# gear-genomics/tracy

Hardware: AMD Instinct MI355X
Metric: GCUPS (tracy align: Gotoh affine-gap DP cells per second, whole job) (higher is better)
Workload: dtype int16 (score sweeps) / int32 (tracebacks)

## Files before the change

### tracy_amd/csrc/capi.hip

```cpp
#include <hip/hip_runtime.h>
#include <atomic>
#include <sched.h>
#include <malloc.h>
#include <map>
#include <chrono>

#include <thread>

#include <algorithm>
#include <cctype>
#include <cstdarg>
#include <cstddef>
#include <cstdio>
#include <cstdlib>
#include <cstring>
#include <string>
#include <memory>
#include <vector>

#include "../../include/tracy_hip.h"
#include "capi_internal.h"
#include "launch.h"
#include "stream_plan.h"
#include "sweep_range.h"
// ... 196 lines not shown
  if (!p.on) return;
  const double ms = (double)(now_ns() - t0) * 1e-6;
  std::lock_guard<std::mutex> lk(p.m);
  auto& e = p.acc[label];
  e.first += ms;
  e.second += 1;
}

namespace {
struct KnobField { const char* name; bool CtxKnobs::*flag; };
const KnobField kKnobFlags[] = {
    {"no_stream", &CtxKnobs::no_stream}, {"no_narrow", &CtxKnobs::no_narrow}, {"no_compact", &CtxKnobs::no_compact},
    {"no_screen", &CtxKnobs::no_screen}, {"no_band", &CtxKnobs::no_band}, {"no_band16", &CtxKnobs::no_band16},
    {"no_front", &CtxKnobs::no_front}, {"no_prefix", &CtxKnobs::no_prefix}, {"no_vote", &CtxKnobs::no_vote},
    {"no_origin", &CtxKnobs::no_origin}, {"no_subwindow", &CtxKnobs::no_subwindow}, {"no_prelim_origin", &CtxKnobs::no_prelim_origin},
    {"no_cq", &CtxKnobs::no_cq}, {"no_fused_walk", &CtxKnobs::no_fused_walk}, {"no_cont16", &CtxKnobs::no_cont16}, {"no_decomp_wave", &CtxKnobs::no_decomp_wave}, {"no_af_split", &CtxKnobs::no_af_split}, {"no_front_lists", &CtxKnobs::no_front_lists}, {"no_origin_band", &CtxKnobs::no_origin_band}, {"no_quads", &CtxKnobs::no_quads}, {"no_fork", &CtxKnobs::no_fork}, {"no_early_tail", &CtxKnobs::no_early_tail}, {"sweeps_alone", &CtxKnobs::sweeps_alone}, {"no_sweep_diag", &CtxKnobs::no_sweep_diag}, {"verbose", &CtxKnobs::verbose}};
bool same_name(const char* a, const char* b) {
  for (; *a && *b; ++a, ++b)
    if (std::tolower((unsigned char)*a) != std::tolower((unsigned char)*b)) return false;
  return *a == *b;
}
}
bool knobs_set(CtxKnobs& k, const char* name, const char* value) {
  if (!name || !value) return false;
  if (same_name(name, "band_w")) {
    char* end = nullptr;
    const long v = strtol(value, &end, 10);
    if (end == value) return false;
    k.band_w = v < 0 ? -1 : (int32_t)std::min<long>(4096, v);
    return true;
  }
  if (same_name(name, "quad_tier_min")) {
    const long v = atol(value);
    if (v < 0) return false;
    k.quad_tier_min = (uint32_t)std::min<long>(v, 0x7fffffffl);
    return true;
  }
  if (same_name(name, "front_list_min")) {
    const long v = atol(value);
    if (v < 0) return false;
    k.front_list_min = (uint32_t)std::min<long>(v, 0x7fffffffl);
    return true;
  }
  if (same_name(name, "b16_multi_max")) {
    char* end = nullptr;
    const long v = strtol(value, &end, 10);
    if (end == value || *end || v < 0 || v > 0x7fffffffl) return false;
    k.b16_multi_max = (uint32_t)v;
    return true;
  }
  if (same_name(name, "chain_prio")) {
    if (value[0] < '0' || value[0] > '2' || value[1]) return false;
// ... 29 lines not shown
      return true;
    }
  return false;
}
void knobs_from_env(CtxKnobs& k) {
  for (const KnobField& f : kKnobFlags) {
    std::string env = "TRACYHIP_";
    for (const char* c = f.name; *c; ++c) env.push_back((char)std::toupper((unsigned char)*c));
    if (getenv(env.c_str())) k.*(f.flag) = true;
  }
  if (getenv("TRACYHIP_HOST_TIMERS")) k.verbose = true;
  if (const char* e = getenv("TRACYHIP_BAND_W")) knobs_set(k, "band_w", e);
  if (const char* e = getenv("TRACYHIP_CKPT_B")) knobs_set(k, "ckpt_b", e);
  if (const char* e = getenv("TRACYHIP_QUAD_TIER_MIN")) knobs_set(k, "quad_tier_min", e);
  if (const char* e = getenv("TRACYHIP_FRONT_LIST_MIN")) knobs_set(k, "front_list_min", e);
  if (const char* e = getenv("TRACYHIP_B16_MULTI_MAX")) knobs_set(k, "b16_multi_max", e);
  if (const char* e = getenv("TRACYHIP_CHAIN_PRIO")) knobs_set(k, "chain_prio", e);
  if (const char* e = getenv("TRACYHIP_SEED_VOTE_CAP")) knobs_set(k, "seed_vote_cap", e);
  if (const char* e = getenv("TRACYHIP_SEED_SPILL")) knobs_set(k, "seed_spill", e);
  if (const char* e = getenv("TRACYHIP_SWEEP_DIAG_PERIOD")) knobs_set(k, "sweep_diag_period", e);
}
std::string knobs_describe(const CtxKnobs& k) {
  std::string s;
  for (const KnobField& f : kKnobFlags) { s += f.name; s += k.*(f.flag) ? "=1\n" : "=0\n"; }
  s += "band_w=" + std::to_string(k.band_w) + "\n";
  s += "ckpt_b=" + std::to_string(k.ckpt_b) + "\n";
  s += "quad_tier_min=" + std::to_string(k.quad_tier_min) + "\n";
  s += "front_list_min=" + std::to_string(k.front_list_min) + "\n";
  s += "b16_multi_max=" + std::to_string(k.b16_multi_max) + "\n";
  s += "chain_prio=" + std::to_string(k.chain_prio) + "\n";
  s += "seed_vote_cap=" + std::to_string(k.seed_vote_cap) + "\n";
  s += k.seed_spill ? "seed_spill=1\n" : "seed_spill=0\n";
  s += "sweep_diag_period=" + std::to_string(k.sweep_diag_period) + "\n";
  s += "host_threads=" + std::to_string(host_pool_threads()) + "\n";
  return s;
}

int timing_begin(tracyhip_ctx* ctx, int which, uint64_t cells, uint64_t bytes) {
  if (!ctx->timing) return TRACYHIP_OK;
  tracyhip_ctx::Pending p{which, nullptr, nullptr, cells, bytes};
  HIP_TRY(get_event(ctx, &p.e0));
  HIP_TRY(get_event(ctx, &p.e1));
  HIP_TRY(hipEventRecord(p.e0, ctx->stream));
// ... 702 lines not shown
      b += (uint64_t)kFrontRows + pre[i].n + 4ull * pre[i].n;
    }
    cells[tid] = c; bytes[tid] = b;
  });
  HIP_TRY(ctx->dev[DB_PRE].ensure(sizeof(PairDesc) * np));
  HIP_TRY(hipMemcpyAsync(ctx->dev[DB_PRE].p, hd, sizeof(PairDesc) * np, hipMemcpyHostToDevice, st));
  DpArgs a = scoring_args(ctx, prm);
  a.pairs = static_cast<const PairDesc*>(ctx->dev[DB_PRE].p);
  a.a1 = d_a1; a.a2 = d_a2; a.scores = nullptr;
  a.special_blocks = d_special;
  a.lastrow = d_lastrow;
  uint64_t tc = 0, tb = 0;
  for (uint32_t t = 0; t < kHostThreads; ++t) { tc += cells[t]; tb += bytes[t]; }
  int trc;
  if ((trc = timing_begin(ctx, TRACYHIP_TIMER_SCORE, tc, tb))) return trc;
  HIP_TRY(launch_gotoh_front_prefix_cq(a, (uint32_t)np, st));
  if ((trc = timing_end(ctx))) return trc;
  return TRACYHIP_OK;
}

static int run_front_once(tracyhip_ctx* ctx, const std::vector<FrontDesc>& fd, const int16_t* d_qp, const uint32_t* d_row, const tracyhip_params* prm,
                          FrontResult& out, const uint8_t* d_codes, bool keep_err, int KB, int32_t halfw) {
  hipStream_t st = ctx->stream;
  const size_t nf = fd.size();
  out.fo.assign(nf, FrontOut{});
  out.score.assign(nf, 0);
  out.ce.assign(nf, 0);
  if (nf == 0) return TRACYHIP_OK;
  const size_t per = sizeof(FrontDesc) + sizeof(PairDesc) + sizeof(FrontOut) + sizeof(int32_t) + 2 * sizeof(uint32_t);
  HIP_TRY(ctx->dev[DB_FRONT].ensure(per * nf + 64));
  PairDesc* d_pairs = static_cast<PairDesc*>(ctx->dev[DB_FRONT].p);
// ... 201 lines not shown
    const uint32_t npre = pre_done ? 0u : (uint32_t)np;
    const uint32_t prows = front_shape ? kFrontRows : (uint32_t)kPrefixLanes * (uint32_t)K;
    uint32_t maxm = 0;
    if (ctx->timing) {
      uint64_t cells = 0, bytes = 0;
      for (size_t i = lo; i < hi; ++i) { cells += (uint64_t)hd[i].m * hd[i].n; bytes += 24ull * hd[i].m + hd[i].n + 4; }
      for (size_t i = 0; i < npre; ++i) cells += (uint64_t)std::min<uint32_t>(hd[nf + i].m, prows) * hd[nf + i].n;
      if ((trc = timing_begin(ctx, TRACYHIP_TIMER_SCORE, cells, bytes))) return trc;
    }
    for (size_t i = lo; i < hi; ++i) { maxm = std::max(maxm, hd[i].m); max_mn = std::max<uint64_t>(max_mn, (uint64_t)hd[i].m + hd[i].n); }
    for (size_t i = 0; i < npre; ++i) max_mn = std::max<uint64_t>(max_mn, (uint64_t)hd[nf + i].m + hd[nf + i].n);
    DpArgs af = a;
    af.pairs = static_cast<const PairDesc*>(ctx->dev[DB_DESC].p) + lo;
    DpArgs apl = ap;
    launch_diag_periods(ctx, prm, K, (uint32_t)(hi - lo), npre, front_shape, af, apl);
    if (front_shape) HIP_TRY(launch_gotoh_ckpt_front(K, af, (uint32_t)(hi - lo), apl, npre, st));
    else HIP_TRY(launch_gotoh_ckpt_prefix(K, af, (uint32_t)(hi - lo), apl, npre, st));
    if ((trc = timing_end(ctx))) return trc;
    if (hi > lo) narrow_launches.emplace_back(maxm, narrow_launch_diag(K, af.diag_period));
    if (npre) narrow_launches.emplace_back(prows, narrow_launch_diag(front_shape ? kFrontPrefixK : K, apl.diag_period));
    pre_done = true;
    lo = hi;
  }
  int32_t herr[kErrWords] = {};
  HIP_TRY(hipMemcpyAsync(herr, ctx->dev[DB_ERR].p, sizeof(herr), hipMemcpyDeviceToHost, st));
  HIP_TRY(ctx_sync(ctx));
  timing_collect(ctx);
  return range_verdict(prm, herr, narrow_launches, max_mn, 0);
}
}

// ... 458 lines not shown
```

### tracy_amd/csrc/capi_internal.h

```cpp
#ifndef TRACY_AMD_CAPI_INTERNAL_H
#define TRACY_AMD_CAPI_INTERNAL_H

#include <hip/hip_runtime.h>

#include <atomic>
#include <condition_variable>
#include <deque>
#include <functional>
#include <mutex>
#include <string>
#include <thread>
#include <utility>
#include <vector>

#include "../../include/tracy_hip.h"
#include "assemble_wave.h"
#include "dp_kernels.h"
#include "band16_launch.h"
#include "front.h"

namespace tracyhip {

struct DevBuf {
  void* p = nullptr;
// ... 185 lines not shown
  bool no_sweep_diag = false;
  bool no_origin_band = false;
  bool no_front_lists = false;
  bool no_af_split = false;
  bool no_decomp_wave = false;
  bool no_cont16 = false;
  bool verbose = false;
  int32_t band_w = -1;
  uint32_t ckpt_b = 256;
  uint32_t chain_prio = 1;
  uint32_t sweep_diag_period = 0;
  uint32_t b16_multi_max = TRACY_B16_MULTI_MAX;
  uint32_t front_list_min = 1024;
  uint32_t seed_vote_cap = 2048;
  bool seed_spill = false;
  uint32_t quad_tier_min = 32768;
};
void knobs_from_env(CtxKnobs& k);
bool knobs_set(CtxKnobs& k, const char* name, const char* value);
std::string knobs_describe(const CtxKnobs& k);

constexpr size_t kCodePad = 128;
int choose_k(uint32_t m, int mode, bool needle = false);
uint64_t seqset_extent(const tracyhip_seqset& s);

struct DpProblem {
  int mode = MODE_CHAR;
  bool a1_profile = false, a2_profile = false;
  const void* d_a1 = nullptr;
  const void* d_a2 = nullptr;
// ... 259 lines not shown
```

### tracy_amd/csrc/dp_kernels.hip

```cpp
#include <hip/hip_runtime.h>

#include <cstdlib>

#include "dp_kernels.h"
#include "launch.h"

namespace tracyhip {

static uint32_t lds_pad() {
  static int v = -1;
  if (v < 0) { const char* e = getenv("TRACYHIP_LDS_PAD"); v = e ? atoi(e) : 0; }
  return (uint32_t)v;
}

struct DeviceWave {
  __device__ __forceinline__ uint32_t lane() const { return threadIdx.x; }
  __device__ __forceinline__ int32_t shift_up(int32_t x) const {
    return __builtin_amdgcn_update_dpp(0, x, 0x138, 0xf, 0xf, true);
  }
  __device__ __forceinline__ int32_t shift_up_row(int32_t x) const {
    return __builtin_amdgcn_update_dpp(0, x, 0x111, 0xf, 0xf, true);
  }
  __device__ __forceinline__ int32_t shift_up_or(int32_t x, int32_t first) const {
    return __builtin_amdgcn_update_dpp(first, x, 0x138, 0xf, 0xf, false);
// ... 487 lines not shown
    if (full.special_blocks) {                                                                                          \
      hipLaunchKernelGGL((gotoh_ckpt_prefix_kernel<KK, GL, true>), grid, dim3(64), lds_combo(KK, true), s, full, nfull, pre, npre); \
      hipLaunchKernelGGL((gotoh_ckpt_prefix_kernel<KK, GL, false>), grid, dim3(64), lds_combo(KK, false), s, full, nfull, pre, npre); \
    } else {                                                                                                            \
      hipLaunchKernelGGL((gotoh_ckpt_prefix_kernel<KK, GL, false>), grid, dim3(64), lds_combo(KK, false), s, full, nfull, pre, npre); \
    }                                                                                                                   \
    break;
  switch (K) {
    TRACY_COMBO_CASE(4) TRACY_COMBO_CASE(8) TRACY_COMBO_CASE(12) TRACY_COMBO_CASE(15) TRACY_COMBO_CASE(16)
    default: return hipErrorInvalidValue;
  }
#undef TRACY_COMBO_CASE
  return hipGetLastError();
}

static uint32_t front_prefix_tall_min() {
  static const uint32_t v = [] { const char* e = getenv("TRACYHIP_PREFIX_TALL_MIN"); return e ? (uint32_t)strtoul(e, nullptr, 10) : 40000u; }();
  return v;
}
template <int GL, int KP>
static hipError_t launch_gotoh_ckpt_front_t(int K, const DpArgs& full, uint32_t nfull, const DpArgs& pre, uint32_t npre, hipStream_t s) {
  static_assert(GL * KP == (int)kFrontRows, "the rows above the kept one");
  const dim3 grid(nfull + (npre + 64 / GL - 1) / (64 / GL));
  auto lds = [](int KK, bool compact) {
    const uint32_t pre_b = lds_bytes_prefix(KP, compact), sw = lds_bytes_sweep16(KK, compact);
    return (pre_b > sw ? pre_b : sw) + lds_pad();
  };
#define TRACY_FRONT_CASE(KK)                                                                                            \
  case KK:                                                                                                              \
    if constexpr (KK == 15 || KK == 16) {                                                                               \
      if (combo_uses_diag<KK>(full, nfull, pre, npre)) {                                                                \
        if (full.special_blocks)                                                                                        \
          hipLaunchKernelGGL((gotoh_ckpt_prefix_kernel<KK, GL, true, KP, true>), grid, dim3(64), lds(KK, true), s, full, nfull, pre, npre); \
        hipLaunchKernelGGL((gotoh_ckpt_prefix_kernel<KK, GL, false, KP, true>), grid, dim3(64), lds(KK, false), s, full, nfull, pre, npre); \
// ... 4 lines not shown
       \
       \
      hipLaunchKernelGGL((gotoh_ckpt_prefix_kernel<KK, GL, true, KP>), grid, dim3(64), lds(KK, true), s, full, nfull, pre, npre); \
      hipLaunchKernelGGL((gotoh_ckpt_prefix_kernel<KK, GL, false, KP>), grid, dim3(64), lds(KK, false), s, full, nfull, pre, npre); \
    } else {                                                                                                            \
      hipLaunchKernelGGL((gotoh_ckpt_prefix_kernel<KK, GL, false, KP>), grid, dim3(64), lds(KK, false), s, full, nfull, pre, npre); \
    }                                                                                                                   \
    break;
  switch (K) {
    TRACY_FRONT_CASE(4) TRACY_FRONT_CASE(8) TRACY_FRONT_CASE(12) TRACY_FRONT_CASE(15) TRACY_FRONT_CASE(16)
    default: return hipErrorInvalidValue;
  }
#undef TRACY_FRONT_CASE
  return hipGetLastError();
}
hipError_t launch_gotoh_ckpt_front(int K, const DpArgs& full, uint32_t nfull, const DpArgs& pre, uint32_t npre, hipStream_t s) {
  if (nfull + npre == 0) return hipSuccess;
  if (nfull == 0 && npre >= front_prefix_tall_min()) return launch_gotoh_ckpt_front_t<(int)kFrontRows / 16, 16>(K, full, nfull, pre, npre, s);
  return launch_gotoh_ckpt_front_t<kFrontPrefixLanes, kFrontPrefixK>(K, full, nfull, pre, npre, s);
}

hipError_t launch_gotoh_prefix(int K, const DpArgs& a, uint32_t npairs, hipStream_t s) {
  if (npairs == 0) return hipSuccess;
  constexpr int GL = kPrefixLanes;
  const dim3 grid((npairs + 64 / GL - 1) / (64 / GL));
#define TRACY_PREFIX_CASE(KK) \
  case KK:                                                                                                                      \
    hipLaunchKernelGGL((gotoh_prefix_kernel<KK, GL, false>), grid, dim3(64), lds_bytes_prefix(KK, false), s, a, npairs);                        \
    if (a.special_blocks) hipLaunchKernelGGL((gotoh_prefix_kernel<KK, GL, true>), grid, dim3(64), lds_bytes_prefix(KK, true), s, a, npairs); \
    break;
  switch (K) {
    TRACY_PREFIX_CASE(4) TRACY_PREFIX_CASE(8) TRACY_PREFIX_CASE(12) TRACY_PREFIX_CASE(15) TRACY_PREFIX_CASE(16)
    default: return hipErrorInvalidValue;
  }
#undef TRACY_PREFIX_CASE
  return hipGetLastError();
}
template <int GL, int KP>
static hipError_t launch_gotoh_front_prefix_cq_t(const DpArgs& a, uint32_t npairs, hipStream_t s) {
  const dim3 grid((npairs + 64 / GL - 1) / (64 / GL));
  hipLaunchKernelGGL((gotoh_prefix_kernel<KP, GL, false, true>), grid, dim3(64), lds_bytes_prefix(KP, false), s, a, npairs);
  if (a.special_blocks) hipLaunchKernelGGL((gotoh_prefix_kernel<KP, GL, true, true>), grid, dim3(64), lds_bytes_prefix(KP, true), s, a, npairs);
  return hipGetLastError();
}
hipError_t launch_gotoh_front_prefix_cq(const DpArgs& a, uint32_t npairs, hipStream_t s) {
  if (npairs == 0) return hipSuccess;
  if (npairs >= front_prefix_tall_min()) return launch_gotoh_front_prefix_cq_t<(int)kFrontRows / 16, 16>(a, npairs, s);
  return launch_gotoh_front_prefix_cq_t<kFrontPrefixLanes, kFrontPrefixK>(a, npairs, s);
}
hipError_t launch_gotoh_walk(const WalkArgs& a, hipStream_t s) {
  if (a.npairs == 0) return hipSuccess;
  hipLaunchKernelGGL(gotoh_walk_kernel, dim3(a.npairs), dim3(64), 0, s, a);
  return hipGetLastError();
}
hipError_t launch_needle_walk(const WalkArgs& a, const uint32_t* bits32, hipStream_t s) {
  if (a.npairs == 0) return hipSuccess;
  hipLaunchKernelGGL(needle_walk_kernel, dim3((a.npairs + 63) / 64), dim3(64), 0, s, a, bits32);
  return hipGetLastError();
}
hipError_t launch_alignment_rows(const RowsArgs& a, hipStream_t s) {
  if (a.npairs == 0) return hipSuccess;
  hipLaunchKernelGGL(alignment_rows_kernel, dim3(a.npairs), dim3(64), 0, s, a);
// ... 5 lines not shown
```

### tracy_amd/csrc/launch.h

```cpp
#ifndef TRACY_AMD_LAUNCH_H
#define TRACY_AMD_LAUNCH_H

#include <hip/hip_runtime.h>

#include "dp_kernels.h"

namespace tracyhip {

struct RowsArgs {
  const PairDesc* pairs;
  const void* a1;
  const void* a2;
  int32_t a1_profile, a2_profile;
  int32_t a2_revcomp_flag;
  int32_t a2_onehot;
  const uint8_t* ops;
  const uint64_t* ops_off;
  const uint32_t* ops_len;
  uint8_t* rows0;
  uint8_t* rows1;
  uint32_t npairs;
  const int32_t* row0_gaps_only;
  uint32_t row0_gaps_only_stride;
};

hipError_t launch_gotoh(int mode, int K, bool trace, bool narrow, const DpArgs& a, uint32_t npairs, hipStream_t s, bool rawtab = false);
hipError_t launch_gotoh_front_prefix_cq(const DpArgs& a, uint32_t npairs, hipStream_t s);
hipError_t launch_gotoh_prof(int K, bool trace, bool row4_zero, bool arith16, const DpArgs& a, uint32_t npairs, hipStream_t s);
hipError_t launch_gotoh_ckpt(int mode, int K, bool narrow, const DpArgs& a, uint32_t npairs, hipStream_t s);
hipError_t launch_band_trace(int mode, int K, const DpArgs& a, const WalkArgs& wa, uint32_t npairs, hipStream_t s);
hipError_t launch_gotoh_origin(int K, int table, int codes, const DpArgs& a, uint32_t npairs, hipStream_t s);
hipError_t launch_gotoh_ckpt_prefix(int K, const DpArgs& full, uint32_t nfull, const DpArgs& pre, uint32_t npre, hipStream_t s);
hipError_t launch_gotoh_prefix(int K, const DpArgs& a, uint32_t npairs, hipStream_t s);
hipError_t launch_gotoh_ckpt_front(int K, const DpArgs& full, uint32_t nfull, const DpArgs& pre, uint32_t npre, hipStream_t s);
hipError_t launch_needle(int mode, int K, bool trace, const DpArgs& a, uint32_t npairs, hipStream_t s);
hipError_t launch_gotoh_walk(const WalkArgs& a, hipStream_t s);
hipError_t launch_needle_walk(const WalkArgs& a, const uint32_t* bits32, hipStream_t s);
hipError_t launch_alignment_rows(const RowsArgs& a, hipStream_t s);

}
#endif
```

### tracy_amd/csrc/stream.hip

```cpp
#include <hip/hip_runtime.h>

#include <algorithm>
#include <cstring>
#include <numeric>
#include <string>
#include <type_traits>
#include <vector>

#include "../../include/tracy_hip.h"
#include "capi_internal.h"
#include "decompose_launch.h"
#include "launch.h"
#include "pipe_internal.h"
#include "pipe_kernels.h"
#include "stream_fields.h"
#include "stream_plan.h"

using namespace tracyhip;

#define TRY(expr) do { const int _rc = (expr); if (_rc) return _rc; } while (0)

namespace {

struct Arena {
// ... 236 lines not shown
      q.n = sw.n;
      q.a2_stride = sw.n;
      q.a2_off = G.ref_off + (S.rc ? (uint64_t)(G.rn - ce) : (uint64_t)sw.a);
      q.flags = S.rc ? PAIR_A2_REVCOMP : 0u;
      q.out = t;
      q.ckpt_off = band_pack(sw.dlo, sw.dhi);
      q.lastrow_off = mode == 0 ? 0ull : ((uint64_t)(G.rn - ce) | ((uint64_t)sw.a << 32));
      cand[t] = q;
      kc[t] = (uint8_t)K;
    }
  }
  tr[t] = S;
  if (dd) dead[t] |= dd;
}

constexpr uint32_t kScanBlock = 256, kScanTop = 1024;
struct ScanPart { uint32_t n[4]; unsigned long long bytes; };
__device__ __forceinline__ int s_bucket(int K, const PairDesc& d, int quads) {
  return K == 12 ? 0 : K == 8 ? 1 : (quads && b16_narrow_ok(band_dmin(d), band_dmax(d))) ? 3 : 2;
}
__device__ __forceinline__ unsigned long long s_word_bytes(const PairDesc& d, int K, int kind, unsigned long long* words = nullptr) {
  if (words) *words = b16_words(d.m, d.n, K, band_dmin(d), band_dmax(d));
  return kind == 0 ? ((b16_store_words(d.m, d.n, K, band_dmin(d), band_dmax(d)) * b16_word_bytes(K) + 15ull) & ~15ull) : 0ull;
}
__global__ __launch_bounds__(kScanBlock) void s_scan_partial_kernel(const PairDesc* __restrict__ cand, const uint8_t* __restrict__ kc, uint32_t n, int kind,
                                                                    int quads, ScanPart* __restrict__ part, int prio) {
  wave_prio(prio);
  __shared__ uint32_t s_n[4];
  __shared__ unsigned long long s_b;
  if (threadIdx.x < 4) s_n[threadIdx.x] = 0;
  if (threadIdx.x == 4) s_b = 0;
  __syncthreads();
  const uint32_t i = blockIdx.x * kScanBlock + threadIdx.x;
  const int K = i < n ? kc[i] : 0;
  if (K) {
    const PairDesc d = cand[i];
    atomicAdd(&s_n[s_bucket(K, d, quads)], 1u);
    if (kind == 0) atomicAdd(&s_b, s_word_bytes(d, K, kind));
  }
  __syncthreads();
  if (threadIdx.x == 0) part[blockIdx.x] = ScanPart{{s_n[0], s_n[1], s_n[2], s_n[3]}, s_b};
}
__global__ __launch_bounds__(kScanTop) void s_scan_top_kernel(ScanPart* __restrict__ part, uint32_t nb, uint32_t* __restrict__ count,
                                                              unsigned long long* __restrict__ stat, int prio) {
  wave_prio(prio);
  __shared__ uint32_t s_n[4][kScanTop];
  __shared__ unsigned long long s_b[kScanTop];
  const uint32_t tid = threadIdx.x;
  const uint32_t per = (nb + kScanTop - 1) / kScanTop;
  const uint32_t lo = tid * per < nb ? tid * per : nb, hi = lo + per < nb ? lo + per : nb;
  uint32_t c[4] = {0, 0, 0, 0};
  unsigned long long bytes = 0;
  for (uint32_t i = lo; i < hi; ++i) { for (int b = 0; b < 4; ++b) c[b] += part[i].n[b]; bytes += part[i].bytes; }
  for (int b = 0; b < 4; ++b) s_n[b][tid] = c[b];
  s_b[tid] = bytes;
  __syncthreads();
  for (uint32_t d = 1; d < kScanTop; d <<= 1) {
    uint32_t v[4] = {0, 0, 0, 0};
    unsigned long long vb = 0;
    if (tid >= d) { for (int b = 0; b < 4; ++b) v[b] = s_n[b][tid - d]; vb = s_b[tid - d]; }
    __syncthreads();
    for (int b = 0; b < 4; ++b) s_n[b][tid] += v[b];
    s_b[tid] += vb;
    __syncthreads();
  }
  uint32_t at[4];
  for (int b = 0; b < 4; ++b) at[b] = s_n[b][tid] - c[b];
  unsigned long long off = s_b[tid] - bytes;
  for (uint32_t i = lo; i < hi; ++i) {
    const ScanPart x = part[i];
    part[i] = ScanPart{{at[0], at[1], at[2], at[3]}, off};
    for (int b = 0; b < 4; ++b) at[b] += x.n[b];
    off += x.bytes;
  }
  if (tid == 0)
    for (int b = 0; b < 4; ++b) {
      count[b] = s_n[b][kScanTop - 1];
      stat[SB_LIST + b] += s_n[b][kScanTop - 1];
    }
}
__global__ __launch_bounds__(kScanBlock) void s_scan_place_kernel(PairDesc* __restrict__ cand, uint8_t* __restrict__ kc, uint32_t n, uint32_t unit_mod, int kind,
                                                                  int quads, unsigned long long cap_bytes, const ScanPart* __restrict__ part, uint32_t* __restrict__ idx,
                                                                  uint32_t* __restrict__ dead, unsigned long long* __restrict__ stat, int prio) {
  wave_prio(prio);
  __shared__ uint32_t s_n[4][kScanBlock];
  __shared__ unsigned long long s_b[kScanBlock];
  __shared__ unsigned long long s_stat[SB_LIST];
  const uint32_t tid = threadIdx.x;
  if (tid < SB_LIST) s_stat[tid] = 0;
  const uint32_t i = blockIdx.x * kScanBlock + tid;
  const int K = i < n ? kc[i] : 0;
  PairDesc d{};
  unsigned long long words = 0, mine = 0;
  if (K) { d = cand[i]; mine = s_word_bytes(d, K, kind, &words); }
  const int bucket = K ? s_bucket(K, d, quads) : -1;
  for (int b = 0; b < 4; ++b) s_n[b][tid] = bucket == b ? 1u : 0u;
  s_b[tid] = mine;
  __syncthreads();
  for (uint32_t dd = 1; dd < kScanBlock; dd <<= 1) {
    uint32_t v[4] = {0, 0, 0, 0};
    unsigned long long vb = 0;
    if (tid >= dd) { for (int b = 0; b < 4; ++b) v[b] = s_n[b][tid - dd]; vb = s_b[tid - dd]; }
    __syncthreads();
    for (int b = 0; b < 4; ++b) s_n[b][tid] += v[b];
    s_b[tid] += vb;
    __syncthreads();
  }
  if (K) {
    const ScanPart base = part[blockIdx.x];
    const int b = bucket;
    const uint32_t pos = base.n[b] + s_n[b][tid] - 1u;
    const unsigned long long off = base.bytes + s_b[tid] - mine;
    idx[(size_t)b * n + pos] = i;
    if (off + mine > cap_bytes) {
      kc[i] = 0;
      cand[i].flags = d.flags | PAIR_SKIP;
      atomicOr(dead + (i % unit_mod), SD_MEM);
    } else {
      cand[i].bits_off = off;
      atomicAdd(&s_stat[0], words * (unsigned long long)K);
      atomicAdd(&s_stat[1], (kind == 0 ? words * b16_word_bytes(K) : 0ull) + 12ull * d.m + d.n + 4ull);
      atomicAdd(&s_stat[2], mine);
      atomicAdd(&s_stat[SB_HIST + s_width_bucket(band_dmin(d), band_dmax(d))], 1ull);
    }
  }
  __syncthreads();
  if (tid < SB_LIST && s_stat[tid]) atomicAdd(stat + tid, s_stat[tid]);
// ... 25 lines not shown
    PairDesc q{};
    q.a1_off = G.tab_off;
    q.a1_stride = G.tab_stride;
    q.m = m;
    q.n = n;
    q.a2_stride = n;
    q.a2_off = G.ref_off + (S.rc ? G.rn - S.trim.ri - S.trim.len : S.trim.ri);
    q.flags = S.rc ? PAIR_A2_REVCOMP : 0u;
    q.out = t;
    q.ckpt_off = band_pack(fb.dlo, fb.dhi);
    cand[t] = q;
    kc[t] = (uint8_t)fb.K;
    s_count(lc, SC_FINAL_BANDED);
    if (early) S.mark |= ST_COUNTED_FINAL;
  }
  tr[t] = S;
  if (dd) dead[t] |= dd;
  });
}

struct AlignOutDev {
  int32_t *score_fwd, *score_rev, *score_prelim, *score_final;
  uint8_t* forward;
  uint32_t *slice_begin, *slice_len, *ref_pos, *ops_len;
};
__global__ void s_align_finish_kernel(SParams p, const STrace* __restrict__ tr, const int32_t* __restrict__ top_full, uint32_t* __restrict__ dead,
                                      AlignOutDev o, unsigned long long* __restrict__ cnt) {
  with_counters(cnt, [&](unsigned long long* lc) {
  const uint32_t t = blockIdx.x * blockDim.x + threadIdx.x;
  if (t >= p.nt) return;
  if (dead[t]) return;
// ... 278 lines not shown
  const uint8_t* codes = nullptr;
  int32_t* scores = nullptr;
  uint32_t* ends = nullptr;
  uint8_t* ops = nullptr;
  const uint64_t* ops_off = nullptr;
  uint32_t* ops_len = nullptr;
  uint32_t code_cap = 0;
  int hfree = 1;
};
int band_stage(tracyhip_ctx* ctx, const tracyhip_params& p, StreamCommon& sc, uint32_t n, uint32_t unit_mod, int stage_no, const BandLaunch& bl, uint64_t cap_bytes) {
  hipStream_t st = ctx->stream;
  uint32_t* count = sc.count + 4 * stage_no;
  const uint32_t nb = (n + kScanBlock - 1) / kScanBlock;
  const int quads = (!ctx->knobs.no_quads && b16_quad_lds(bl.code_cap) <= 64u * 1024u) ? 1 : 0;
  const int prio = queued_prio(ctx, 2);
  hipLaunchKernelGGL(s_scan_partial_kernel, dim3(nb), dim3(kScanBlock), 0, st, sc.cand, sc.kc, n, bl.kind, quads, sc.part, prio);
  hipLaunchKernelGGL(s_scan_top_kernel, dim3(1), dim3(kScanTop), 0, st, sc.part, nb, count, sc.bstat + SB_COUNT * stage_no, prio);
  hipLaunchKernelGGL(s_scan_place_kernel, dim3(nb), dim3(kScanBlock), 0, st, sc.cand, sc.kc, n, unit_mod, bl.kind, quads, (unsigned long long)cap_bytes, sc.part, sc.idx, sc.dead,
                     sc.bstat + SB_COUNT * stage_no, prio);
  HIP_TRY(hipGetLastError());
  Band16Args a{};
  a.prio = prio;
  a.pairs = sc.cand; a.npairs = n; a.qp = bl.qp; a.codes = bl.codes; a.bits = static_cast<uint8_t*>(ctx->dev[DB_BITS].p); a.scores = bl.scores; a.ends = bl.ends;
  a.err = static_cast<int32_t*>(ctx->dev[DB_ERR].p); a.go = p.go; a.ge = p.ge; a.hfree = bl.hfree;
  a.ops = bl.ops; a.ops_off = bl.ops_off; a.ops_len = bl.ops_len; a.code_cap = bl.code_cap;
  Band16Args ak[4] = {a, a, a, a};
  for (int b = 0; b < 4; ++b) { ak[b].index = sc.idx + (size_t)b * n; ak[b].count = count + b; }
  if (!quads) ak[3].npairs = 0;
  TRY(timing_begin(ctx, bl.kind == 0 ? TRACYHIP_TIMER_TRACE : TRACYHIP_TIMER_ORIGIN, 0, 0));
  bool large = false;
  HIP_TRY(launch_band16_counted(bl.kind, ak[0], ak[1], ak[2], ak[3], st, (ctx->b16_fork_ok && !ctx->knobs.no_fork) ? &ctx->b16_fork : nullptr,
                                ctx->knobs.b16_multi_max, &large));
  if (large) ++sc.large_stages;
  TRY(timing_end(ctx));
// ... 60 lines not shown
  auto front_tiers = [&]() -> int {
    TRY(timing_begin(ctx, TRACYHIP_TIMER_FRONT, 0, 0));
    const int rc = front_tiers_run(ctx, p, sc, nt, os.d_qp, ctx->codes(), reinterpret_cast<const uint32_t*>(os.d_lastrow), h.max_rest);
    const int rc2 = timing_end(ctx);
    return rc ? rc : rc2;
  };
  if (ctx->b16_fork_ok && !ctx->knobs.no_fork) {
    const B16Fork& fk = ctx->b16_fork;
    HIP_TRY(hipEventRecord(fk.forked, st));
    HIP_TRY(hipStreamWaitEvent(fk.side[0], fk.forked, 0));
    ctx->stream = fk.side[0];
    int rc = TRACYHIP_OK;
    {
      DpArgs af = a, apl = ap;
      launch_diag_periods(ctx, &p, h.classes[0].K, 0u, npre_all, true, af, apl);
      if (launch_gotoh_ckpt_front(h.classes[0].K, af, 0u, apl, npre_all, fk.side[0]) != hipSuccess) rc = set_error(TRACYHIP_ERR_HIP, "prefix launch failed");
    }
    ctx->queue_prio = ctx->knobs.chain_prio;
    if (!rc) rc = front_tiers();
    if (!rc && os.early_tail) {
      hipLaunchKernelGGL(s_orient_early_kernel, g256, b256, 0, fk.side[0], sp, sc.fo1, sc.fs1, sc.fe1, sc.fo2, sc.fs2, sc.fe2, sc.tr, queued_prio(ctx, 1));
      if (hipGetLastError() != hipSuccess) rc = set_error(TRACYHIP_ERR_HIP, "early decision launch failed");
      else rc = os.early_tail();
    }
    ctx->queue_prio = 0;
    ctx->stream = st;
    HIP_TRY(hipEventRecord(fk.joined[0], fk.side[0]));
    if (rc) {
      HIP_TRY(hipStreamWaitEvent(st, fk.joined[0], 0));
      return rc;
    }
    if (ctx->knobs.sweeps_alone) HIP_TRY(hipStreamWaitEvent(st, fk.joined[0], 0));
    auto sweeps = [&]() -> int {
      for (const SweepClass& c : h.classes) {
        DpArgs af = a;
        af.pairs = sc.full + 2 * (size_t)c.lo;
        DpArgs apl = ap;
        launch_diag_periods(ctx, &p, c.K, 2 * (c.hi - c.lo), 0u, true, af, apl);
        TRY(timing_begin(ctx, TRACYHIP_TIMER_SCORE, 0, 0));
        const hipError_t e = launch_gotoh_ckpt_front(c.K, af, 2 * (c.hi - c.lo), apl, 0u, st);
        TRY(timing_end(ctx));
        HIP_TRY(e);
      }
      return os.filler ? os.filler() : TRACYHIP_OK;
    };
    const int src = sweeps();
    HIP_TRY(hipStreamWaitEvent(st, fk.joined[0], 0));
    if (src) return src;
  } else {
    bool pre_done = false;
    for (const SweepClass& c : h.classes) {
      DpArgs af = a;
      af.pairs = sc.full + 2 * (size_t)c.lo;
      DpArgs apl = ap;
      launch_diag_periods(ctx, &p, c.K, 2 * (c.hi - c.lo), pre_done ? 0u : npre_all, true, af, apl);
      TRY(timing_begin(ctx, TRACYHIP_TIMER_SCORE, 0, 0));
      HIP_TRY(launch_gotoh_ckpt_front(c.K, af, 2 * (c.hi - c.lo), apl, pre_done ? 0u : npre_all, st));
      TRY(timing_end(ctx));
      pre_done = true;
    }
    TRY(front_tiers());
  }
  hipLaunchKernelGGL(s_orient_decide_kernel, g256, b256, 0, st, sp, sc.geom, sc.votes, sc.ub, sc.sc2, sc.fo1, sc.fs1, sc.fe1, sc.fo2, sc.fs2, sc.fe2, sc.tr, sc.re,
                     sc.dead, sc.cnt, os.desc_trim);
  hipLaunchKernelGGL(row_m_end_kernel, dim3(nt), dim3(64), 0, st, static_cast<const RowEndDesc*>(sc.re), static_cast<const int32_t*>(os.d_lastrow), p.go + p.ge, sc.ce);
  HIP_TRY(hipGetLastError());
  return TRACYHIP_OK;
}

struct PlanHooks {
  std::function<void(uint32_t lo, uint32_t hi, uint32_t tid)> lengths_slice;
  std::function<int()> between;
// ... 1184 lines not shown
    HIP_TRY(hipGetLastError());
    if (share) {
      HIP_TRY(hipMemsetAsync(sc.fcount + 2, 0, sizeof(uint32_t), st));
      hipLaunchKernelGGL(s_pair_list_kernel, g256x2, b256, 0, st, 2 * nt, sc.pre, sc.flist, sc.fcount + 2);
      HIP_TRY(hipGetLastError());
    }
    {
      DpArgs a = scoring_args(ctx, &p);
      a.pairs = sc.pre;
      if (share) { a.index = sc.flist; a.count = sc.fcount + 2; }
      a.a1 = A.seqs2; a.a2 = d_cq_ref;
      a.special_blocks = kn.no_compact ? nullptr : A.cq_special;
      a.lastrow = d_lastrow;
      if (af_pending) HIP_TRY(hipEventRecord(ctx->b16_fork.ready[0], st));
      TRY(timing_begin(ctx, TRACYHIP_TIMER_SCORE, 0, 0));
      HIP_TRY(launch_gotoh_front_prefix_cq(a, 2 * nt, st));
      TRY(timing_end(ctx));
    }
    if (af_pending) TRY(give_up(queue_allelic_fraction()));
    TRY(timing_begin(ctx, TRACYHIP_TIMER_FRONT, 0, 0));
    {
      int rc = front_tiers_run(ctx, p, sc, 2 * nt, d_aqp, d_cq_ref, reinterpret_cast<const uint32_t*>(d_lastrow), max_arest);
      if (rc) return give_up(rc);
    }
    TRY(timing_end(ctx));
    hipLaunchKernelGGL(s_allele_plan1_kernel, g256x2, b256, 0, st, spm, spd, sc.geom, A.geomd, sc.tr, sc.fo1, sc.fs1, sc.fe1, sc.fo2, sc.fs2, sc.fe2, A.al, sc.dead, sc.cand,
                       sc.kc, sc.cnt);
    HIP_TRY(hipGetLastError());
    BandLaunch b1;
    b1.kind = 1; b1.qp = d_aqp; b1.codes = d_cq_ref; b1.ends = sc.ends; b1.code_cap = ncap; b1.hfree = 1;
    TRY(band_stage(ctx, p, sc, 2 * nt, nt, 1, b1, ~0ull));
// ... 97 lines not shown
```

Before: 19080.

## Replace three-kernel band scan with wave-ballot count/place, force tall prefix beside sweeps

The band-stage compaction drops the single-block top-level scan kernel. Per-block counts now come from wave ballots and shuffles, and each place block sums the preceding block partials itself, so there is one fewer launch and no serial 1024-thread scan. The prefix tall-variant threshold moves from a static env read into a context knob, and the forked prefix launch in exact mode always uses the tall variant. Trace-state writes now store only the three fields that change instead of the whole struct. Each place block re-reads all earlier partials, which costs quadratic reads when the block count is large.

```diff
diff --git a/tracy_amd/csrc/capi.hip b/tracy_amd/csrc/capi.hip
--- a/tracy_amd/csrc/capi.hip
+++ b/tracy_amd/csrc/capi.hip
@@ -234,7 +234,7 @@
     {"no_screen", &CtxKnobs::no_screen}, {"no_band", &CtxKnobs::no_band}, {"no_band16", &CtxKnobs::no_band16},
     {"no_front", &CtxKnobs::no_front}, {"no_prefix", &CtxKnobs::no_prefix}, {"no_vote", &CtxKnobs::no_vote},
     {"no_origin", &CtxKnobs::no_origin}, {"no_subwindow", &CtxKnobs::no_subwindow}, {"no_prelim_origin", &CtxKnobs::no_prelim_origin},
-    {"no_cq", &CtxKnobs::no_cq}, {"no_fused_walk", &CtxKnobs::no_fused_walk}, {"no_cont16", &CtxKnobs::no_cont16}, {"no_decomp_wave", &CtxKnobs::no_decomp_wave}, {"no_af_split", &CtxKnobs::no_af_split}, {"no_front_lists", &CtxKnobs::no_front_lists}, {"no_origin_band", &CtxKnobs::no_origin_band}, {"no_quads", &CtxKnobs::no_quads}, {"no_fork", &CtxKnobs::no_fork}, {"no_early_tail", &CtxKnobs::no_early_tail}, {"sweeps_alone", &CtxKnobs::sweeps_alone}, {"no_sweep_diag", &CtxKnobs::no_sweep_diag}, {"verbose", &CtxKnobs::verbose}};
+    {"no_cq", &CtxKnobs::no_cq}, {"no_fused_walk", &CtxKnobs::no_fused_walk}, {"no_cont16", &CtxKnobs::no_cont16}, {"no_decomp_wave", &CtxKnobs::no_decomp_wave}, {"no_af_split", &CtxKnobs::no_af_split}, {"no_front_lists", &CtxKnobs::no_front_lists}, {"no_origin_band", &CtxKnobs::no_origin_band}, {"no_quads", &CtxKnobs::no_quads}, {"no_fork", &CtxKnobs::no_fork}, {"no_early_tail", &CtxKnobs::no_early_tail}, {"sweeps_alone", &CtxKnobs::sweeps_alone}, {"no_sweep_diag", &CtxKnobs::no_sweep_diag}, {"no_prefix_tall_beside", &CtxKnobs::no_prefix_tall_beside}, {"verbose", &CtxKnobs::verbose}};
 bool same_name(const char* a, const char* b) {
   for (; *a && *b; ++a, ++b)
     if (std::tolower((unsigned char)*a) != std::tolower((unsigned char)*b)) return false;
@@ -256,6 +256,13 @@
     k.quad_tier_min = (uint32_t)std::min<long>(v, 0x7fffffffl);
     return true;
   }
+  if (same_name(name, "prefix_tall_min")) {
+    char* end = nullptr;
+    const long v = strtol(value, &end, 10);
+    if (end == value || *end || v < 0 || v > 0x7fffffffl) return false;
+    k.prefix_tall_min = (uint32_t)v;
+    return true;
+  }
   if (same_name(name, "front_list_min")) {
     const long v = atol(value);
     if (v < 0) return false;
@@ -315,6 +322,7 @@
   if (const char* e = getenv("TRACYHIP_CKPT_B")) knobs_set(k, "ckpt_b", e);
   if (const char* e = getenv("TRACYHIP_QUAD_TIER_MIN")) knobs_set(k, "quad_tier_min", e);
   if (const char* e = getenv("TRACYHIP_FRONT_LIST_MIN")) knobs_set(k, "front_list_min", e);
+  if (const char* e = getenv("TRACYHIP_PREFIX_TALL_MIN")) knobs_set(k, "prefix_tall_min", e);
   if (const char* e = getenv("TRACYHIP_B16_MULTI_MAX")) knobs_set(k, "b16_multi_max", e);
   if (const char* e = getenv("TRACYHIP_CHAIN_PRIO")) knobs_set(k, "chain_prio", e);
   if (const char* e = getenv("TRACYHIP_SEED_VOTE_CAP")) knobs_set(k, "seed_vote_cap", e);
@@ -328,6 +336,7 @@
   s += "ckpt_b=" + std::to_string(k.ckpt_b) + "\n";
   s += "quad_tier_min=" + std::to_string(k.quad_tier_min) + "\n";
   s += "front_list_min=" + std::to_string(k.front_list_min) + "\n";
+  s += "prefix_tall_min=" + std::to_string(k.prefix_tall_min) + "\n";
   s += "b16_multi_max=" + std::to_string(k.b16_multi_max) + "\n";
   s += "chain_prio=" + std::to_string(k.chain_prio) + "\n";
   s += "seed_vote_cap=" + std::to_string(k.seed_vote_cap) + "\n";
@@ -1060,7 +1069,7 @@
   for (uint32_t t = 0; t < kHostThreads; ++t) { tc += cells[t]; tb += bytes[t]; }
   int trc;
   if ((trc = timing_begin(ctx, TRACYHIP_TIMER_SCORE, tc, tb))) return trc;
-  HIP_TRY(launch_gotoh_front_prefix_cq(a, (uint32_t)np, st));
+  HIP_TRY(launch_gotoh_front_prefix_cq(a, (uint32_t)np, st, ctx->knobs.prefix_tall_min));
   if ((trc = timing_end(ctx))) return trc;
   return TRACYHIP_OK;
 }
@@ -1292,7 +1301,7 @@
     af.pairs = static_cast<const PairDesc*>(ctx->dev[DB_DESC].p) + lo;
     DpArgs apl = ap;
     launch_diag_periods(ctx, prm, K, (uint32_t)(hi - lo), npre, front_shape, af, apl);
-    if (front_shape) HIP_TRY(launch_gotoh_ckpt_front(K, af, (uint32_t)(hi - lo), apl, npre, st));
+    if (front_shape) HIP_TRY(launch_gotoh_ckpt_front(K, af, (uint32_t)(hi - lo), apl, npre, st, ctx->knobs.prefix_tall_min));
     else HIP_TRY(launch_gotoh_ckpt_prefix(K, af, (uint32_t)(hi - lo), apl, npre, st));
     if ((trc = timing_end(ctx))) return trc;
     if (hi > lo) narrow_launches.emplace_back(maxm, narrow_launch_diag(K, af.diag_period));
diff --git a/tracy_amd/csrc/capi_internal.h b/tracy_amd/csrc/capi_internal.h
--- a/tracy_amd/csrc/capi_internal.h
+++ b/tracy_amd/csrc/capi_internal.h
@@ -223,6 +223,8 @@
   uint32_t front_list_min = 1024;
   uint32_t seed_vote_cap = 2048;
   bool seed_spill = false;
+  bool no_prefix_tall_beside = false;
+  uint32_t prefix_tall_min = 40000;
   uint32_t quad_tier_min = 32768;
 };
 void knobs_from_env(CtxKnobs& k);
diff --git a/tracy_amd/csrc/dp_kernels.hip b/tracy_amd/csrc/dp_kernels.hip
--- a/tracy_amd/csrc/dp_kernels.hip
+++ b/tracy_amd/csrc/dp_kernels.hip
@@ -525,10 +525,6 @@
   return hipGetLastError();
 }
 
-static uint32_t front_prefix_tall_min() {
-  static const uint32_t v = [] { const char* e = getenv("TRACYHIP_PREFIX_TALL_MIN"); return e ? (uint32_t)strtoul(e, nullptr, 10) : 40000u; }();
-  return v;
-}
 template <int GL, int KP>
 static hipError_t launch_gotoh_ckpt_front_t(int K, const DpArgs& full, uint32_t nfull, const DpArgs& pre, uint32_t npre, hipStream_t s) {
   static_assert(GL * KP == (int)kFrontRows, "the rows above the kept one");
@@ -563,9 +559,9 @@
 #undef TRACY_FRONT_CASE
   return hipGetLastError();
 }
-hipError_t launch_gotoh_ckpt_front(int K, const DpArgs& full, uint32_t nfull, const DpArgs& pre, uint32_t npre, hipStream_t s) {
+hipError_t launch_gotoh_ckpt_front(int K, const DpArgs& full, uint32_t nfull, const DpArgs& pre, uint32_t npre, hipStream_t s, uint32_t tall_min) {
   if (nfull + npre == 0) return hipSuccess;
-  if (nfull == 0 && npre >= front_prefix_tall_min()) return launch_gotoh_ckpt_front_t<(int)kFrontRows / 16, 16>(K, full, nfull, pre, npre, s);
+  if (nfull == 0 && npre >= tall_min) return launch_gotoh_ckpt_front_t<(int)kFrontRows / 16, 16>(K, full, nfull, pre, npre, s);
   return launch_gotoh_ckpt_front_t<kFrontPrefixLanes, kFrontPrefixK>(K, full, nfull, pre, npre, s);
 }
 
@@ -592,9 +588,9 @@
   if (a.special_blocks) hipLaunchKernelGGL((gotoh_prefix_kernel<KP, GL, true, true>), grid, dim3(64), lds_bytes_prefix(KP, true), s, a, npairs);
   return hipGetLastError();
 }
-hipError_t launch_gotoh_front_prefix_cq(const DpArgs& a, uint32_t npairs, hipStream_t s) {
-  if (npairs == 0) return hipSuccess;
-  if (npairs >= front_prefix_tall_min()) return launch_gotoh_front_prefix_cq_t<(int)kFrontRows / 16, 16>(a, npairs, s);
+hipError_t launch_gotoh_front_prefix_cq(const DpArgs& a, uint32_t npairs, hipStream_t s, uint32_t tall_min) {
+  if (npairs == 0) return hipSuccess;
+  if (npairs >= tall_min) return launch_gotoh_front_prefix_cq_t<(int)kFrontRows / 16, 16>(a, npairs, s);
   return launch_gotoh_front_prefix_cq_t<kFrontPrefixLanes, kFrontPrefixK>(a, npairs, s);
 }
 hipError_t launch_gotoh_walk(const WalkArgs& a, hipStream_t s) {
diff --git a/tracy_amd/csrc/launch.h b/tracy_amd/csrc/launch.h
--- a/tracy_amd/csrc/launch.h
+++ b/tracy_amd/csrc/launch.h
@@ -25,14 +25,14 @@
 };
 
 hipError_t launch_gotoh(int mode, int K, bool trace, bool narrow, const DpArgs& a, uint32_t npairs, hipStream_t s, bool rawtab = false);
-hipError_t launch_gotoh_front_prefix_cq(const DpArgs& a, uint32_t npairs, hipStream_t s);
+hipError_t launch_gotoh_front_prefix_cq(const DpArgs& a, uint32_t npairs, hipStream_t s, uint32_t tall_min);
 hipError_t launch_gotoh_prof(int K, bool trace, bool row4_zero, bool arith16, const DpArgs& a, uint32_t npairs, hipStream_t s);
 hipError_t launch_gotoh_ckpt(int mode, int K, bool narrow, const DpArgs& a, uint32_t npairs, hipStream_t s);
 hipError_t launch_band_trace(int mode, int K, const DpArgs& a, const WalkArgs& wa, uint32_t npairs, hipStream_t s);
 hipError_t launch_gotoh_origin(int K, int table, int codes, const DpArgs& a, uint32_t npairs, hipStream_t s);
 hipError_t launch_gotoh_ckpt_prefix(int K, const DpArgs& full, uint32_t nfull, const DpArgs& pre, uint32_t npre, hipStream_t s);
 hipError_t launch_gotoh_prefix(int K, const DpArgs& a, uint32_t npairs, hipStream_t s);
-hipError_t launch_gotoh_ckpt_front(int K, const DpArgs& full, uint32_t nfull, const DpArgs& pre, uint32_t npre, hipStream_t s);
+hipError_t launch_gotoh_ckpt_front(int K, const DpArgs& full, uint32_t nfull, const DpArgs& pre, uint32_t npre, hipStream_t s, uint32_t tall_min);
 hipError_t launch_needle(int mode, int K, bool trace, const DpArgs& a, uint32_t npairs, hipStream_t s);
 hipError_t launch_gotoh_walk(const WalkArgs& a, hipStream_t s);
 hipError_t launch_needle_walk(const WalkArgs& a, const uint32_t* bits32, hipStream_t s);
diff --git a/tracy_amd/csrc/stream.hip b/tracy_amd/csrc/stream.hip
--- a/tracy_amd/csrc/stream.hip
+++ b/tracy_amd/csrc/stream.hip
@@ -274,7 +274,7 @@
   if (dd) dead[t] |= dd;
 }
 
-constexpr uint32_t kScanBlock = 256, kScanTop = 1024;
+constexpr uint32_t kScanBlock = 256, kScanWaves = kScanBlock / 64;
 struct ScanPart { uint32_t n[4]; unsigned long long bytes; };
 __device__ __forceinline__ int s_bucket(int K, const PairDesc& d, int quads) {
   return K == 12 ? 0 : K == 8 ? 1 : (quads && b16_narrow_ok(band_dmin(d), band_dmax(d))) ? 3 : 2;
@@ -283,94 +283,93 @@
   if (words) *words = b16_words(d.m, d.n, K, band_dmin(d), band_dmax(d));
   return kind == 0 ? ((b16_store_words(d.m, d.n, K, band_dmin(d), band_dmax(d)) * b16_word_bytes(K) + 15ull) & ~15ull) : 0ull;
 }
-__global__ __launch_bounds__(kScanBlock) void s_scan_partial_kernel(const PairDesc* __restrict__ cand, const uint8_t* __restrict__ kc, uint32_t n, int kind,
-                                                                    int quads, ScanPart* __restrict__ part, int prio) {
+__device__ __forceinline__ uint32_t s_wave_sum(uint32_t v) {
+  for (int o = 32; o > 0; o >>= 1) v += (uint32_t)__shfl_xor((int)v, o, 64);
+  return v;
+}
+__device__ __forceinline__ unsigned long long s_wave_sum(unsigned long long v) {
+  for (int o = 32; o > 0; o >>= 1) v += __shfl_xor(v, o, 64);
+  return v;
+}
+__device__ __forceinline__ ScanPart s_waves_before(const ScanPart* __restrict__ w, uint32_t upto) {
+  ScanPart t{{0, 0, 0, 0}, 0};
+  for (uint32_t k = 0; k < upto; ++k) { for (int b = 0; b < 4; ++b) t.n[b] += w[k].n[b]; t.bytes += w[k].bytes; }
+  return t;
+}
+__global__ __launch_bounds__(kScanBlock) void s_scan_count_kernel(const PairDesc* __restrict__ cand, const uint8_t* __restrict__ kc, uint32_t n, int kind,
+                                                                  int quads, ScanPart* __restrict__ part, int prio) {
   wave_prio(prio);
-  __shared__ uint32_t s_n[4];
-  __shared__ unsigned long long s_b;
-  if (threadIdx.x < 4) s_n[threadIdx.x] = 0;
-  if (threadIdx.x == 4) s_b = 0;
-  __syncthreads();
-  const uint32_t i = blockIdx.x * kScanBlock + threadIdx.x;
+  __shared__ ScanPart s_w[kScanWaves];
+  const uint32_t tid = threadIdx.x, wv = tid >> 6, L = tid & 63u;
+  const uint32_t i = blockIdx.x * kScanBlock + tid;
   const int K = i < n ? kc[i] : 0;
+  int bucket = -1;
+  unsigned long long mine = 0;
   if (K) {
     const PairDesc d = cand[i];
-    atomicAdd(&s_n[s_bucket(K, d, quads)], 1u);
-    if (kind == 0) atomicAdd(&s_b, s_word_bytes(d, K, kind));
-  }
+    bucket = s_bucket(K, d, quads);
+    mine = s_word_bytes(d, K, kind);
+  }
+  ScanPart w;
+  for (int b = 0; b < 4; ++b) w.n[b] = (uint32_t)__popcll(__ballot(bucket == b));
+  w.bytes = s_wave_sum(mine);
+  if (L == 0) s_w[wv] = w;
   __syncthreads();
-  if (threadIdx.x == 0) part[blockIdx.x] = ScanPart{{s_n[0], s_n[1], s_n[2], s_n[3]}, s_b};
-}
-__global__ __launch_bounds__(kScanTop) void s_scan_top_kernel(ScanPart* __restrict__ part, uint32_t nb, uint32_t* __restrict__ count,
-                                                              unsigned long long* __restrict__ stat, int prio) {
-  wave_prio(prio);
-  __shared__ uint32_t s_n[4][kScanTop];
-  __shared__ unsigned long long s_b[kScanTop];
-  const uint32_t tid = threadIdx.x;
-  const uint32_t per = (nb + kScanTop - 1) / kScanTop;
-  const uint32_t lo = tid * per < nb ? tid * per : nb, hi = lo + per < nb ? lo + per : nb;
-  uint32_t c[4] = {0, 0, 0, 0};
-  unsigned long long bytes = 0;
-  for (uint32_t i = lo; i < hi; ++i) { for (int b = 0; b < 4; ++b) c[b] += part[i].n[b]; bytes += part[i].bytes; }
-  for (int b = 0; b < 4; ++b) s_n[b][tid] = c[b];
-  s_b[tid] = bytes;
-  __syncthreads();
-  for (uint32_t d = 1; d < kScanTop; d <<= 1) {
-    uint32_t v[4] = {0, 0, 0, 0};
-    unsigned long long vb = 0;
-    if (tid >= d) { for (int b = 0; b < 4; ++b) v[b] = s_n[b][tid - d]; vb = s_b[tid - d]; }
-    __syncthreads();
-    for (int b = 0; b < 4; ++b) s_n[b][tid] += v[b];
-    s_b[tid] += vb;
-    __syncthreads();
-  }
-  uint32_t at[4];
-  for (int b = 0; b < 4; ++b) at[b] = s_n[b][tid] - c[b];
-  unsigned long long off = s_b[tid] - bytes;
-  for (uint32_t i = lo; i < hi; ++i) {
-    const ScanPart x = part[i];
-    part[i] = ScanPart{{at[0], at[1], at[2], at[3]}, off};
-    for (int b = 0; b < 4; ++b) at[b] += x.n[b];
-    off += x.bytes;
-  }
-  if (tid == 0)
-    for (int b = 0; b < 4; ++b) {
-      count[b] = s_n[b][kScanTop - 1];
-      stat[SB_LIST + b] += s_n[b][kScanTop - 1];
-    }
+  if (tid == 0) part[blockIdx.x] = s_waves_before(s_w, kScanWaves);
 }
 __global__ __launch_bounds__(kScanBlock) void s_scan_place_kernel(PairDesc* __restrict__ cand, uint8_t* __restrict__ kc, uint32_t n, uint32_t unit_mod, int kind,
                                                                   int quads, unsigned long long cap_bytes, const ScanPart* __restrict__ part, uint32_t* __restrict__ idx,
-                                                                  uint32_t* __restrict__ dead, unsigned long long* __restrict__ stat, int prio) {
+                                                                  uint32_t* __restrict__ dead, uint32_t* __restrict__ count, unsigned long long* __restrict__ stat,
+                                                                  int prio) {
   wave_prio(prio);
-  __shared__ uint32_t s_n[4][kScanBlock];
-  __shared__ unsigned long long s_b[kScanBlock];
+  __shared__ ScanPart s_base[kScanWaves];
+  __shared__ ScanPart s_w[kScanWaves];
   __shared__ unsigned long long s_stat[SB_LIST];
-  const uint32_t tid = threadIdx.x;
+  const uint32_t tid = threadIdx.x, wv = tid >> 6, L = tid & 63u;
   if (tid < SB_LIST) s_stat[tid] = 0;
+  ScanPart before{{0, 0, 0, 0}, 0};
+  for (uint32_t j = tid; j < blockIdx.x; j += kScanBlock) {
+    const ScanPart x = part[j];
+    for (int b = 0; b < 4; ++b) before.n[b] += x.n[b];
+    before.bytes += x.bytes;
+  }
+  for (int b = 0; b < 4; ++b) before.n[b] = s_wave_sum(before.n[b]);
+  before.bytes = s_wave_sum(before.bytes);
   const uint32_t i = blockIdx.x * kScanBlock + tid;
   const int K = i < n ? kc[i] : 0;
   PairDesc d{};
   unsigned long long words = 0, mine = 0;
   if (K) { d = cand[i]; mine = s_word_bytes(d, K, kind, &words); }
   const int bucket = K ? s_bucket(K, d, quads) : -1;
-  for (int b = 0; b < 4; ++b) s_n[b][tid] = bucket == b ? 1u : 0u;
-  s_b[tid] = mine;
+  const unsigned long long below = (1ull << L) - 1ull;
+  ScanPart w;
+  uint32_t rank = 0;
+  for (int b = 0; b < 4; ++b) {
+    const unsigned long long bal = __ballot(bucket == b);
+    w.n[b] = (uint32_t)__popcll(bal);
+    if (bucket == b) rank = (uint32_t)__popcll(bal & below);
+  }
+  unsigned long long incl = mine;
+  for (int o = 1; o < 64; o <<= 1) {
+    const unsigned long long y = __shfl_up(incl, o, 64);
+    if (L >= (uint32_t)o) incl += y;
+  }
+  w.bytes = __shfl(incl, 63, 64);
+  if (L == 0) { s_base[wv] = before; s_w[wv] = w; }
   __syncthreads();
-  for (uint32_t dd = 1; dd < kScanBlock; dd <<= 1) {
-    uint32_t v[4] = {0, 0, 0, 0};
-    unsigned long long vb = 0;
-    if (tid >= dd) { for (int b = 0; b < 4; ++b) v[b] = s_n[b][tid - dd]; vb = s_b[tid - dd]; }
-    __syncthreads();
-    for (int b = 0; b < 4; ++b) s_n[b][tid] += v[b];
-    s_b[tid] += vb;
-    __syncthreads();
+  const ScanPart base = s_waves_before(s_base, kScanWaves), lower = s_waves_before(s_w, wv);
+  if (blockIdx.x == gridDim.x - 1 && tid == 0) {
+    const ScanPart all = s_waves_before(s_w, kScanWaves);
+    for (int b = 0; b < 4; ++b) {
+      count[b] = base.n[b] + all.n[b];
+      stat[SB_LIST + b] += base.n[b] + all.n[b];
+    }
   }
   if (K) {
-    const ScanPart base = part[blockIdx.x];
     const int b = bucket;
-    const uint32_t pos = base.n[b] + s_n[b][tid] - 1u;
-    const unsigned long long off = base.bytes + s_b[tid] - mine;
+    uint32_t pos = rank;
+    for (int k = 0; k < 4; ++k) pos += b == k ? base.n[k] + lower.n[k] : 0u;
+    const unsigned long long off = base.bytes + lower.bytes + incl - mine;
     idx[(size_t)b * n + pos] = i;
     if (off + mine > cap_bytes) {
       kc[i] = 0;
@@ -426,7 +425,9 @@
     s_count(lc, SC_FINAL_BANDED);
     if (early) S.mark |= ST_COUNTED_FINAL;
   }
-  tr[t] = S;
+  tr[t].bw = S.bw;
+  tr[t].mark = S.mark;
+  tr[t].trim = S.trim;
   if (dd) dead[t] |= dd;
   });
 }
@@ -735,10 +736,9 @@
   const uint32_t nb = (n + kScanBlock - 1) / kScanBlock;
   const int quads = (!ctx->knobs.no_quads && b16_quad_lds(bl.code_cap) <= 64u * 1024u) ? 1 : 0;
   const int prio = queued_prio(ctx, 2);
-  hipLaunchKernelGGL(s_scan_partial_kernel, dim3(nb), dim3(kScanBlock), 0, st, sc.cand, sc.kc, n, bl.kind, quads, sc.part, prio);
-  hipLaunchKernelGGL(s_scan_top_kernel, dim3(1), dim3(kScanTop), 0, st, sc.part, nb, count, sc.bstat + SB_COUNT * stage_no, prio);
+  hipLaunchKernelGGL(s_scan_count_kernel, dim3(nb), dim3(kScanBlock), 0, st, sc.cand, sc.kc, n, bl.kind, quads, sc.part, prio);
   hipLaunchKernelGGL(s_scan_place_kernel, dim3(nb), dim3(kScanBlock), 0, st, sc.cand, sc.kc, n, unit_mod, bl.kind, quads, (unsigned long long)cap_bytes, sc.part, sc.idx, sc.dead,
-                     sc.bstat + SB_COUNT * stage_no, prio);
+                     count, sc.bstat + SB_COUNT * stage_no, prio);
   HIP_TRY(hipGetLastError());
   Band16Args a{};
   a.prio = prio;
@@ -829,7 +829,8 @@
     {
       DpArgs af = a, apl = ap;
       launch_diag_periods(ctx, &p, h.classes[0].K, 0u, npre_all, true, af, apl);
-      if (launch_gotoh_ckpt_front(h.classes[0].K, af, 0u, apl, npre_all, fk.side[0]) != hipSuccess) rc = set_error(TRACYHIP_ERR_HIP, "prefix launch failed");
+      const uint32_t tall_min = (os.exact && !ctx->knobs.no_prefix_tall_beside) ? 0u : ctx->knobs.prefix_tall_min;
+      if (launch_gotoh_ckpt_front(h.classes[0].K, af, 0u, apl, npre_all, fk.side[0], tall_min) != hipSuccess) rc = set_error(TRACYHIP_ERR_HIP, "prefix launch failed");
     }
     ctx->queue_prio = ctx->knobs.chain_prio;
     if (!rc) rc = front_tiers();
@@ -853,7 +854,7 @@
         DpArgs apl = ap;
         launch_diag_periods(ctx, &p, c.K, 2 * (c.hi - c.lo), 0u, true, af, apl);
         TRY(timing_begin(ctx, TRACYHIP_TIMER_SCORE, 0, 0));
-        const hipError_t e = launch_gotoh_ckpt_front(c.K, af, 2 * (c.hi - c.lo), apl, 0u, st);
+        const hipError_t e = launch_gotoh_ckpt_front(c.K, af, 2 * (c.hi - c.lo), apl, 0u, st, ctx->knobs.prefix_tall_min);
         TRY(timing_end(ctx));
         HIP_TRY(e);
       }
@@ -870,7 +871,7 @@
       DpArgs apl = ap;
       launch_diag_periods(ctx, &p, c.K, 2 * (c.hi - c.lo), pre_done ? 0u : npre_all, true, af, apl);
       TRY(timing_begin(ctx, TRACYHIP_TIMER_SCORE, 0, 0));
-      HIP_TRY(launch_gotoh_ckpt_front(c.K, af, 2 * (c.hi - c.lo), apl, pre_done ? 0u : npre_all, st));
+      HIP_TRY(launch_gotoh_ckpt_front(c.K, af, 2 * (c.hi - c.lo), apl, pre_done ? 0u : npre_all, st, ctx->knobs.prefix_tall_min));
       TRY(timing_end(ctx));
       pre_done = true;
     }
@@ -2085,7 +2086,7 @@
       a.lastrow = d_lastrow;
       if (af_pending) HIP_TRY(hipEventRecord(ctx->b16_fork.ready[0], st));
       TRY(timing_begin(ctx, TRACYHIP_TIMER_SCORE, 0, 0));
-      HIP_TRY(launch_gotoh_front_prefix_cq(a, 2 * nt, st));
+      HIP_TRY(launch_gotoh_front_prefix_cq(a, 2 * nt, st, ctx->knobs.prefix_tall_min));
       TRY(timing_end(ctx));
     }
     if (af_pending) TRY(give_up(queue_allelic_fraction()));
```

Result: faster. 19520 (median of 6 runs) (+2.3%).
